# tari-project/bulletproofs-plus

Measured on AMD Instinct MI355X. Metric: 64-bit range proofs verified/sec (batch), higher is better.
Workload: dtype u32

## Files before the change

bulletproofs-plus_amd/csrc/engine.hip:

```cpp
#include <hip/hip_runtime.h>
#include <errno.h>
#include <sched.h>
#include <stdio.h>
#include <string.h>
#include <time.h>

#include <algorithm>
#include <atomic>
#include <chrono>
#include <condition_variable>
#include <deque>
#include <functional>
#include <map>
#include <set>
#include <memory>
#include <mutex>
#include <string>
#include <thread>
#include <vector>

#include "../../include/bpp.h"
#include "chain_dev.h"
#include "chain_host.h"
#include "ct.h"
// ... 323 lines not shown
    uint32_t cap = 0;
    while ((2u << cap) <= std::max<uint32_t>(max_mn, 1)) cap++;
    const uint32_t rm = std::min({rmax, (uint32_t)BPP_MAX_ROUNDS - 1, cap}), lb = lanes_lb(n_bits);
    return 1u << (rm > lb ? rm - lb : 0);
  }
  std::vector<ProofDesc> desc;
  std::vector<uint8_t> rounds_bad;
  std::vector<uint8_t> defer;
  bool any_seed = false, any_rounds_bad = false, any_defer = false, ext_challenges = false, uniform_rounds = true;
  std::vector<uint32_t> ext_status;
  DevBuf<uint32_t> d_ext_status;
  DevBuf<uint8_t> bytes, states, seeds;
  DevBuf<ProofDesc> d_desc;
  DevBuf<uint64_t> minvals;
  DevBuf<uint32_t> src_off, owner;
  DevBuf<uint32_t> idx_commit, idx_proof, status0;
  DevBuf<sc> chal, rows, scal, shr, tab;
  DevBuf<uint64_t> parts;
  bool fused_columns = false;
  uint32_t lanes_ppw = 1;
  DevBuf<int8_t> gemm_lo, gemm_hi;
  DevBuf<int32_t> gparts;
  DevBuf<sc> gemm_mult;
  bool static_gemm = false;
  uint32_t gemm_nkc = 1;
  int uniform_mn = -1;
  bool gemm_hi_ready = false;
  DevBuf<uint8_t> rng_out, weights, masks, chal_bytes;
  DevBuf<uint32_t> chain_wide;
  DevBuf<uint32_t> status, group_first, group_dlo;
  DevBuf<uint32_t> dec_spill;
  DevBuf<niels> dynpts;
  DevBuf<pniels> dyn_hi;
  MsmWork msm;
  size_t last_chunk = (size_t)-1;
  uint32_t G = 0;
  std::vector<uint32_t> h_group_first;
  PinnedBuf<uint8_t> h_rng, h_weights, h_masks;
  PinnedBuf<uint8_t> h_wide;
  PinnedBuf<uint32_t> h_status, h_ident;
  PinnedBuf<uint32_t> h_status_any;
  std::vector<uint8_t> h_status_dirty;
  const uint32_t *h_status_dirty_of = nullptr;
  bool status_settled = true;
  bool have_trace = false, phase1_done = false;
  bool status_clean = false;
  bool dev_chain_pending = false;
  bool weights_on_host = false;
  bool seeds_dirty = false, masks_dirty = false;
};

void adopt_buffers(Batch &dst, Batch &src) {
#define BPP_ADOPT(f) dst.f.swap(src.f)
  BPP_ADOPT(d_ext_status); BPP_ADOPT(bytes); BPP_ADOPT(states); BPP_ADOPT(seeds); BPP_ADOPT(d_desc); BPP_ADOPT(minvals);
  BPP_ADOPT(src_off); BPP_ADOPT(owner); BPP_ADOPT(idx_commit); BPP_ADOPT(idx_proof); BPP_ADOPT(status0); BPP_ADOPT(chal);
  BPP_ADOPT(rows); BPP_ADOPT(parts); BPP_ADOPT(gemm_lo); BPP_ADOPT(gemm_hi); BPP_ADOPT(gparts); BPP_ADOPT(gemm_mult); BPP_ADOPT(scal); BPP_ADOPT(shr); BPP_ADOPT(tab); BPP_ADOPT(rng_out); BPP_ADOPT(weights); BPP_ADOPT(chain_wide);
  BPP_ADOPT(masks); BPP_ADOPT(chal_bytes); BPP_ADOPT(status); BPP_ADOPT(group_first); BPP_ADOPT(group_dlo); BPP_ADOPT(dynpts); BPP_ADOPT(dyn_hi); BPP_ADOPT(dec_spill);
  BPP_ADOPT(msm.counts); BPP_ADOPT(msm.starts); BPP_ADOPT(msm.sorted); BPP_ADOPT(msm.order); BPP_ADOPT(msm.order_win);
  BPP_ADOPT(msm.cls_hist);
  BPP_ADOPT(msm.buckets); BPP_ADOPT(msm.Q); BPP_ADOPT(msm.W); BPP_ADOPT(msm.R); BPP_ADOPT(msm.comp32);
  BPP_ADOPT(msm.is_identity); BPP_ADOPT(msm.term_sidx); BPP_ADOPT(msm.term_pidx); BPP_ADOPT(msm.group_off);
  BPP_ADOPT(h_rng); BPP_ADOPT(h_weights); BPP_ADOPT(h_wide); BPP_ADOPT(h_status); BPP_ADOPT(h_status_any); BPP_ADOPT(h_ident); BPP_ADOPT(h_masks);
#undef BPP_ADOPT
  dst.h_status_dirty.swap(src.h_status_dirty);
  std::swap(dst.h_status_dirty_of, src.h_status_dirty_of);
  if (!src.status_settled) std::fill(dst.h_status_dirty.begin(), dst.h_status_dirty.end(), (uint8_t)1);
}

void wipe_batch_secrets(Batch &b, hipStream_t s);

}

struct PipeJob {
  uint64_t ticket = 0;
  int action = 0;
  size_t chunk = 0;
  std::shared_ptr<Params> Pp;
  uint64_t params = 0;
  UploadPlan pl;
  size_t n_items = 0;
  uint32_t t = 0;
  int rc = 0;
  std::string err;
  std::vector<uint8_t> masks, present;
  bool done = false;
};

struct PipeLane {
  bpp_ctx *child = nullptr;
  std::thread th;
  std::shared_ptr<PipeJob> job;
  bool busy = false;
};

struct Pipeline {
  std::mutex mu;
  std::condition_variable cv;
  std::mutex submit_mu;
  std::vector<std::unique_ptr<PipeLane>> lanes;
  std::map<uint64_t, std::shared_ptr<PipeJob>> tickets;
  uint64_t next_ticket = 1;
  uint32_t next_lane = 0;
  bool quit = false;
};

void pipeline_shutdown(bpp_ctx *ctx);

struct WaitHint {
  uint32_t us = 0;
  uint64_t key = 0;
};

struct bpp_ctx {
  int device = 0;
  hipStream_t stream = nullptr;
  bool own_stream = false;
  std::string err;
  std::mutex mu;
  std::multiset<uint64_t> held_params, held_precomps;
  std::map<uint64_t, std::unique_ptr<Batch>> batches;
  std::unique_ptr<Batch> spare_batch;
  PinnedBuf<uint8_t> pin_upload, pin_upload2;
  PinnedBuf<uint32_t> pin_small;
  bool profile = false;
  bool profile_light = false;
  bpp_profile prof{};
  hipEvent_t ev[16];
  bool ev_ready = false;
  hipEvent_t ev_rng;
  bool ev_rng_ready = false;
  hipEvent_t ev_wait;
  bool ev_wait_ready = false;
  WaitHint wait_hint_rng, wait_hint_end, wait_hint_prove;
  hipStream_t side_stream = nullptr;
  hipEvent_t ev_fork, ev_join;
  hipStream_t chain_stream = nullptr;
  hipEvent_t ev_chain_fork, ev_chain_done;
  DevBuf<Strobe> d_chain_t0;
  PinnedBuf<uint32_t> h_chain_zero;
  uint64_t device_chain_calls = 0, device_chain_redraws = 0, wide_chain_calls = 0;
  DevBuf<uint8_t> scratch128;
  DevBuf<uint8_t> prove_arena;
  PinnedBuf<uint8_t> prove_pin_in, prove_pin_out;
  std::vector<hipStream_t> prove_streams;
  std::vector<hipStream_t> prove_lane_streams;
  hipStream_t prove_msm_stream = nullptr;
  std::vector<hipEvent_t> prove_sync_events;
  std::vector<hipStream_t> prove_aux_streams;
  std::vector<hipEvent_t> prove_aux_events;
  std::vector<hipEvent_t> prove_events;
  bpp_prove_profile pprof{};
  struct Options {
    int transcripts_wave = -1, tables_wave = -1, side_decompress = -1, msm_c_bias = -1, msm_c_max = -1, msm_c_add = -1, msm_rc2 = -1, msm_quad = -1, msm_final_quad = -1,
        fb_threads = -1, prove_subs = -1, msm_split = -1, fused_columns = -1, prove_prio = -1, prove_fused = -1, static_gemm = -1, lazy_columns = -1, ct = -1, prove_parts = -1, prove_waves = -1, prove_fifo = -1, chain = -1, chain_test_zero = 0, wait = -1, ct_back = -1, chain_inline = -1, wide_in_lanes = -1;
  } opt;
  std::unique_ptr<Pipeline> pipe;
  std::mutex pipe_init_mu;
  uint32_t pipe_depth = 3;
};

namespace {

static uint32_t fb_threads(const bpp_ctx *ctx, uint32_t terms, const FbGeom &g) {
  if (ctx->opt.fb_threads > 0) {
    const uint32_t t = ((uint32_t)ctx->opt.fb_threads + 63u) & ~63u;
    return t > FB_THREADS ? FB_THREADS : t;
  }
  const uint32_t items = terms * g.windows;
  return items >= 4096 ? 256u : (items >= 1024 ? 128u : 64u);
}

struct OptionName {
  const char *name, *env;
  int bpp_ctx::Options::*field;
};
const OptionName kOptions[] = {
    {"transcripts_wave", "BPP_TRANSCRIPTS_WAVE", &bpp_ctx::Options::transcripts_wave},
    {"tables_wave", "BPP_TABLES_WAVE", &bpp_ctx::Options::tables_wave},
    {"side_decompress", "BPP_SIDE_DECOMPRESS", &bpp_ctx::Options::side_decompress},
    {"msm_c_bias", "BPP_MSM_C_BIAS", &bpp_ctx::Options::msm_c_bias},
    {"msm_c_max", "BPP_MSM_C_MAX", &bpp_ctx::Options::msm_c_max},
    {"msm_c_add", "BPP_MSM_C_ADD", &bpp_ctx::Options::msm_c_add},
    {"msm_rc2", "BPP_MSM_RC2", &bpp_ctx::Options::msm_rc2},
    {"msm_quad", "BPP_MSM_QUAD", &bpp_ctx::Options::msm_quad},
    {"msm_final_quad", "BPP_MSM_FINAL_QUAD", &bpp_ctx::Options::msm_final_quad},
    {"fb_threads", "BPP_FB_THREADS", &bpp_ctx::Options::fb_threads},
    {"prove_subs", "BPP_PROVE_SUBS", &bpp_ctx::Options::prove_subs},
    {"msm_split", "BPP_MSM_SPLIT", &bpp_ctx::Options::msm_split},
    {"fused_columns", "BPP_FUSED_COLUMNS", &bpp_ctx::Options::fused_columns},
    {"prove_prio", "BPP_PROVE_PRIO", &bpp_ctx::Options::prove_prio},
    {"prove_fused", "BPP_PROVE_FUSED", &bpp_ctx::Options::prove_fused},
    {"ct", "BPP_CT", &bpp_ctx::Options::ct},
    {"ct_back", "BPP_CT_BACK", &bpp_ctx::Options::ct_back},
    {"prove_parts", "BPP_PROVE_PARTS", &bpp_ctx::Options::prove_parts},
    {"prove_waves", "BPP_PROVE_WAVES", &bpp_ctx::Options::prove_waves},
    {"prove_fifo", "BPP_PROVE_FIFO", &bpp_ctx::Options::prove_fifo},
    {"static_gemm", "BPP_STATIC_GEMM", &bpp_ctx::Options::static_gemm},
    {"lazy_columns", "BPP_LAZY_COLUMNS", &bpp_ctx::Options::lazy_columns},
    {"chain", "BPP_CHAIN", &bpp_ctx::Options::chain},
    {"chain_test_zero", "BPP_CHAIN_TEST_ZERO", &bpp_ctx::Options::chain_test_zero},
    {"wait", "BPP_WAIT", &bpp_ctx::Options::wait},
    {"chain_inline", "BPP_CHAIN_INLINE", &bpp_ctx::Options::chain_inline},
    {"wide_in_lanes", "BPP_WIDE_IN_LANES", &bpp_ctx::Options::wide_in_lanes},
};
void options_from_env(bpp_ctx *c) {
  for (const OptionName &o : kOptions)
    if (const char *e = getenv(o.env)) c->opt.*(o.field) = atoi(e);
}

int fail(bpp_ctx *ctx, int code, const std::string &m, char *errbuf = nullptr, size_t len = 0) {
  if (ctx) ctx->err = m;
  set_err(errbuf, len, m);
  return code;
}

enum Mark { M_START = 0, M_TRANSCRIPTS, M_DECOMPRESS, M_SCALARS, M_WEIGHTS_IN, M_LANES, M_REDUCE, M_DIGITS, M_SORT, M_ORDER, M_ACC,
            M_BUCKET, M_FINAL, M_MASKS0, M_MASKS, M_CHAIN, M_COUNT };

struct StageTimer {
  bpp_ctx *ctx;
  bool have[16] = {false};
  explicit StageTimer(bpp_ctx *c) : ctx(c) {
    if (ctx->profile && !ctx->ev_ready) {
      for (auto &e : ctx->ev) HIP_CHECK(hipEventCreate(&e));
      ctx->ev_ready = true;
    }
  }
  void mark(int idx) {
    if (ctx->profile && idx < 16) {
      if (ctx->profile_light && idx != M_ORDER && idx != M_ACC) return;
      HIP_CHECK(hipEventRecord(ctx->ev[idx], ctx->stream));
      have[idx] = true;
    }
  }
  float between(int a, int b) {
    float ms = 0;
    if (ctx->profile && have[a] && have[b]) HIP_CHECK(hipEventElapsedTime(&ms, ctx->ev[a], ctx->ev[b]));
    return ms;
  }
};

inline uint32_t cdiv(uint32_t a, uint32_t b) { return (a + b - 1) / b; }

#define BPP_WAIT_NAP_MIN_PROOFS 4096u
inline bool wait_naps(const bpp_ctx *ctx, size_t proofs) {
  return ctx->opt.wait >= 0 ? ctx->opt.wait != 0 : proofs >= BPP_WAIT_NAP_MIN_PROOFS;
}
inline void gpu_wait_event(hipEvent_t ev, bool nap, WaitHint *wh = nullptr, uint64_t key = 0, bool tail_spin = false) {
  if (wh && wh->key != key) {
    wh->us = 0;
    wh->key = key;
  }
  uint32_t *hint = wh ? &wh->us : nullptr;
  if (!nap) {
    HIP_CHECK(hipEventSynchronize(ev));
    return;
  }
  const auto t0 = std::chrono::steady_clock::now();
  bool slept_ahead = false;
  for (;;) {
    const hipError_t e = hipEventQuery(ev);
    const long waited = (long)std::chrono::duration_cast<std::chrono::microseconds>(std::chrono::steady_clock::now() - t0).count();
    if (e == hipSuccess) {
      if (hint) *hint = *hint ? (uint32_t)((3ul * *hint + (unsigned long)waited) / 4ul) : (uint32_t)waited;
      return;
    }
    if (e != hipErrorNotReady) HIP_CHECK(e);
    if (waited < 30) continue;
    if (tail_spin && (slept_ahead || !hint || *hint <= 600)) continue;
    long nap_us;
    if (hint && !slept_ahead && *hint > 600 && waited < (long)*hint / 2) {
      nap_us = (long)*hint * (tail_spin ? 7 : 5) / 10 - waited;
      if (nap_us < 50) nap_us = 50;
      slept_ahead = true;
    } else if (slept_ahead && waited < (long)*hint * 5 / 4) {
      nap_us = 50;
    } else {
      nap_us = waited < 400 ? 50 : (waited / 8 > 400 ? 400 : waited / 8);
    }
    struct timespec ts = {0, nap_us * 1000};
    nanosleep(&ts, nullptr);
  }
}
inline void gpu_wait_stream(bpp_ctx *ctx, hipStream_t s, bool nap, WaitHint *hint = nullptr, uint64_t key = 0, bool tail_spin = false);
inline bool gpu_wait_stream_ok(bpp_ctx *ctx, hipStream_t s, bool nap) {
  try {
    gpu_wait_stream(ctx, s, nap);
    return true;
  } catch (const EngineError &) {
    (void)hipGetLastError();
    return false;
  }
}
inline void gpu_wait_stream(bpp_ctx *ctx, hipStream_t s, bool nap, WaitHint *hint, uint64_t key, bool tail_spin) {
  if (!nap) {
    HIP_CHECK(hipStreamSynchronize(s));
    return;
  }
  if (!ctx->ev_wait_ready) {
    HIP_CHECK(hipEventCreateWithFlags(&ctx->ev_wait, hipEventDisableTiming));
    ctx->ev_wait_ready = true;
  }
  HIP_CHECK(hipEventRecord(ctx->ev_wait, s));
  gpu_wait_event(ctx->ev_wait, true, hint, key, tail_spin);
}

static bool decompress_spill_enabled() {
  static const bool on = [] {
    const char *e = getenv("BPP_DECOMPRESS_SPILL");
    return e ? atoi(e) != 0 : true;
  }();
  return on;
}


#define BPP_SMALL_CALL_TERMS 20000u
uint32_t choose_window(const bpp_ctx *ctx, uint32_t group_terms, uint32_t all_terms) {
  uint32_t c = 4;
  while (c < 14 && (1u << c) * 12u <= group_terms) c++;
  const uint32_t c_max = ctx->opt.msm_c_max >= 0 ? (uint32_t)ctx->opt.msm_c_max : (group_terms < 200000u ? 11u : 14u);
  if (ctx->opt.msm_c_add > 0 && all_terms > BPP_SMALL_CALL_TERMS) c += (uint32_t)ctx->opt.msm_c_add;
  if (c > c_max && c_max >= 4) c = c_max;
  const int bias = ctx->opt.msm_c_bias >= 0 ? ctx->opt.msm_c_bias : 3;
  if (all_terms <= BPP_SMALL_CALL_TERMS) c = (uint32_t)std::max(4, std::min(11, (int)c + bias));
  return c;
}

#define BPP_SPLIT_CALL_TERMS 14000u
bool msm_wants_split(const bpp_ctx *ctx, uint32_t n_terms) {
  if (ctx->opt.msm_split >= 0) return ctx->opt.msm_split != 0 && ctx->opt.msm_quad != 0;
  return n_terms <= BPP_SPLIT_CALL_TERMS && ctx->opt.msm_quad != 0;
}
void msm_plan_alloc(bpp_ctx *ctx, MsmWork &w, const std::vector<uint32_t> &goff, bool split = false, bool copy_goff = true) {
  const uint32_t G = (uint32_t)goff.size() - 1, n = goff[G];
  uint32_t maxg = 0;
  for (uint32_t g = 0; g < G; g++) maxg = std::max(maxg, goff[g + 1] - goff[g]);
  const MsmPlan plan = msm_make_plan(choose_window(ctx, maxg, split ? n / 2 : n), G, n, split ? BPP_MSM_SPLIT_BITS : 253u);
  w.plan = plan;
  w.split = split;
  w.max_group_terms = maxg;
  const size_t nbk = (size_t)G * plan.K * plan.nb;
  w.counts.alloc(nbk);
  w.starts.alloc(nbk);
  w.sorted.alloc((size_t)n * plan.K);
  w.order.alloc(nbk);
  w.order_win.alloc(nbk);
  w.cls_hist.alloc((size_t)G * plan.K * 768);
  w.buckets.alloc(nbk);
  w.Q.alloc((size_t)G * plan.K * plan.c);
  w.W.alloc((size_t)G * plan.K);
  w.R.alloc(G);
  w.comp32.alloc((size_t)G * 32);
  w.is_identity.alloc(G);
  w.term_sidx.alloc(n);
  w.term_pidx.alloc(n);
  w.group_off.alloc(G + 1);
  HIP_CHECK(hipStreamSynchronize(ctx->stream));
  ctx->pin_small.resize(3 * (size_t)(G + 1));
  memcpy(ctx->pin_small.data(), goff.data(), (G + 1) * 4);
  if (copy_goff) HIP_CHECK(hipMemcpyAsync(w.group_off.p, ctx->pin_small.data(), (G + 1) * 4, hipMemcpyHostToDevice, ctx->stream));
}

void msm_prepare(bpp_ctx *ctx, MsmWork &w, const std::vector<uint32_t> &sidx, const std::vector<uint32_t> &pidx,
                 const std::vector<uint32_t> &goff) {
  msm_plan_alloc(ctx, w, goff);
  const uint32_t n = (uint32_t)sidx.size(), G1 = (uint32_t)goff.size();
  HIP_CHECK(hipStreamSynchronize(ctx->stream));
  ctx->pin_small.resize(3 * (size_t)G1 + 2 * (size_t)n);
  uint32_t *pin = ctx->pin_small.data() + 3 * (size_t)G1;
  memcpy(pin, sidx.data(), (size_t)n * 4);
  memcpy(pin + n, pidx.data(), (size_t)n * 4);
  HIP_CHECK(hipMemcpyAsync(w.term_sidx.p, pin, (size_t)n * 4, hipMemcpyHostToDevice, ctx->stream));
  HIP_CHECK(hipMemcpyAsync(w.term_pidx.p, pin + n, (size_t)n * 4, hipMemcpyHostToDevice, ctx->stream));
  HIP_CHECK(hipStreamSynchronize(ctx->stream));
}

void msm_run(bpp_ctx *ctx, MsmWork &w, const sc *scalars, PointTables tabs, StageTimer *tm) {
  const MsmPlan plan = w.plan;
  hipStream_t s = ctx->stream;
  const uint32_t per_group = plan.K * plan.nb;
  const bool small = w.split || (ctx->opt.msm_quad >= 0 ? ctx->opt.msm_quad != 0 : (size_t)plan.G * per_group <= 100000);
  const bool narrow = !small && w.max_group_terms <= BPP_SORT_SMALL_GROUP_TERMS;
  if (narrow) {
    const uint32_t dig_cap = msm_prelude_dig_cap(plan, w.max_group_terms, BPP_SORT_THREADS_SMALL);
    hipLaunchKernelGGL(k_msm_prelude<BPP_SORT_THREADS_SMALL>, dim3(8 * cdiv(plan.G, 8) * plan.K), dim3(BPP_SORT_THREADS_SMALL), msm_prelude_lds(plan, dig_cap), s,
                       scalars, w.term_sidx.p, w.term_pidx.p, w.group_off.p, plan, dig_cap, w.counts.p, w.starts.p, w.sorted.p, w.order_win.p, w.cls_hist.p);
    hipLaunchKernelGGL(k_msm_order<BPP_SORT_THREADS_SMALL>, dim3(plan.G), dim3(BPP_SORT_THREADS_SMALL), 0, s, w.counts.p, w.order_win.p, w.cls_hist.p, plan,
                       w.order.p);
  } else {
    const uint32_t dig_cap = msm_prelude_dig_cap(plan, w.max_group_terms);
    hipLaunchKernelGGL(k_msm_prelude<BPP_SORT_THREADS>, dim3(8 * cdiv(plan.G, 8) * plan.K), dim3(BPP_SORT_THREADS), msm_prelude_lds(plan, dig_cap), s, scalars,
                       w.term_sidx.p, w.term_pidx.p, w.group_off.p, plan, dig_cap, w.counts.p, w.starts.p, w.sorted.p, w.order_win.p, w.cls_hist.p);
    hipLaunchKernelGGL(k_msm_order<BPP_SORT_THREADS>, dim3(plan.G), dim3(BPP_SORT_THREADS), 0, s, w.counts.p, w.order_win.p, w.cls_hist.p, plan, w.order.p);
  }
  if (tm) tm->mark(M_ORDER);
  if (small)
    hipLaunchKernelGGL(k_msm_accumulate_quad, dim3(cdiv(plan.G * per_group, 16)), dim3(64), 0, s, w.sorted.p, w.starts.p,
                       w.counts.p, w.order.p, tabs, plan.G * per_group, w.buckets.p);
  else
    hipLaunchKernelGGL(k_msm_accumulate, dim3(8 * cdiv(plan.G, 8) * cdiv(per_group, 64)), dim3(64), 0, s, w.sorted.p, w.starts.p,
                       w.counts.p, w.order.p, tabs, per_group, plan.G, w.buckets.p);
  if (tm) tm->mark(M_ACC);
  if (plan.c <= 11 && small) {
    hipLaunchKernelGGL(k_msm_window_rc_quad, dim3(plan.G * plan.K), dim3(1024), 0, s, w.buckets.p, w.counts.p, plan, w.W.p);
  } else if (plan.nb <= 256 && ctx->opt.msm_rc2 != 0) {
    hipLaunchKernelGGL(k_msm_window_rc2, dim3(cdiv(plan.G * plan.K, 2)), dim3(64), 0, s, w.buckets.p, w.counts.p, plan, plan.G * plan.K, w.W.p);
  } else if (plan.c <= 11) {
    hipLaunchKernelGGL(k_msm_window_rc, dim3(plan.G * plan.K), dim3(64), 0, s, w.buckets.p, w.counts.p, plan, w.W.p);
  } else {
    hipLaunchKernelGGL(k_msm_bitsum, dim3(plan.c, plan.K, plan.G), dim3(64), 0, s, w.buckets.p, w.counts.p, plan, w.Q.p);
    hipLaunchKernelGGL(k_msm_window, dim3(cdiv(plan.G * plan.K, 64)), dim3(64), 0, s, w.Q.p, plan, w.W.p);
  }
  if (tm) tm->mark(M_BUCKET);
  {
    if (ctx->opt.msm_final_quad != 0)
      hipLaunchKernelGGL(k_msm_final_quad, dim3(cdiv(plan.G, 16)), dim3(64), 0, s, w.W.p, plan, w.R.p, w.is_identity.p);
    else
      hipLaunchKernelGGL(k_msm_final, dim3(cdiv(plan.G, 64)), dim3(64), 0, s, w.W.p, plan, w.R.p, w.is_identity.p);
  }
  if (tm) tm->mark(M_FINAL);
  HIP_CHECK(hipGetLastError());
}

uint32_t decompress_to_device(bpp_ctx *ctx, const uint8_t *pts32, size_t n, niels *out) {
  DevBuf<uint8_t> d_in;
  DevBuf<uint32_t> d_bad;
  d_in.alloc(n * 32);
  d_bad.alloc(1);
  HIP_CHECK(hipMemcpyAsync(d_in.p, pts32, n * 32, hipMemcpyHostToDevice, ctx->stream));
  HIP_CHECK(hipMemsetAsync(d_bad.p, 0, 4, ctx->stream));
  hipLaunchKernelGGL(k_decompress_plain, dim3(cdiv((uint32_t)n, 64)), dim3(64), 0, ctx->stream, d_in.p, (uint32_t)n, out,
                     d_bad.p);
  uint32_t bad = 0;
  HIP_CHECK(hipMemcpyAsync(&bad, d_bad.p, 4, hipMemcpyDeviceToHost, ctx->stream));
  HIP_CHECK(hipStreamSynchronize(ctx->stream));
  return bad;
}

int msm_host_entry(bpp_ctx *ctx, const niels *tab_a, uint32_t n_a, const uint8_t *static_scalars32, size_t n_static,
                   const uint8_t *dyn_scalars32, const uint8_t *dyn_points32, size_t n_dyn,
                   const uint32_t *group_off_in, size_t n_groups, uint8_t *out32) {
  const size_t n = n_static + n_dyn;
  std::vector<uint8_t> sb(n * 32 + 32);
  if (n_static) memcpy(sb.data(), static_scalars32, n_static * 32);
  if (n_dyn) memcpy(sb.data() + n_static * 32, dyn_scalars32, n_dyn * 32);
  for (size_t i = 0; i < n; i++)
    if (!sc_is_canonical(sb.data() + 32 * i)) return fail(ctx, BPP_ERR_INVALID_ARGUMENT, "scalar is not canonical");
  if (n == 0 || n_groups == 0) {
    for (size_t g = 0; g < (n_groups ? n_groups : 1); g++) memset(out32 + 32 * g, 0, 32);
    return BPP_OK;
  }
  DevBuf<sc> d_sc;
  DevBuf<niels> d_dyn;
  d_sc.alloc(n);
  d_dyn.alloc(n_dyn);
  HIP_CHECK(hipMemcpyAsync(d_sc.p, sb.data(), n * 32, hipMemcpyHostToDevice, ctx->stream));
  if (n_dyn) {
    uint32_t bad = decompress_to_device(ctx, dyn_points32, n_dyn, d_dyn.p);
    if (bad) return fail(ctx, BPP_ERR_INVALID_ARGUMENT, "point is not a canonical ristretto255 encoding");
  }
  std::vector<uint32_t> sidx(n), pidx(n), goff;
  for (size_t i = 0; i < n; i++) {
    sidx[i] = (uint32_t)i;
    pidx[i] = (i < n_static) ? (uint32_t)i : (uint32_t)(n_a + (i - n_static));
  }
  if (group_off_in) {
    goff.assign(group_off_in, group_off_in + n_groups + 1);
  } else {
    goff = {0u, (uint32_t)n};
  }
  MsmWork w;
  msm_prepare(ctx, w, sidx, pidx, goff);
  PointTables tabs{tab_a, d_dyn.p, n_a, nullptr, nullptr};
  msm_run(ctx, w, d_sc.p, tabs, nullptr);
  hipLaunchKernelGGL(k_compress_ge, dim3(cdiv(w.plan.G, 64)), dim3(64), 0, ctx->stream, w.R.p, w.plan.G, w.comp32.p);
  HIP_CHECK(hipMemcpyAsync(out32, w.comp32.p, 32 * (goff.size() - 1), hipMemcpyDeviceToHost, ctx->stream));
  HIP_CHECK(hipStreamSynchronize(ctx->stream));
  return BPP_OK;
}

}

extern "C" {

int bpp_ctx_create_on_stream(bpp_ctx **out, int device_id, void *hip_stream) {
  if (!out) return BPP_ERR_BAD_HANDLE;
  *out = nullptr;
  int count = 0;
  if (hipGetDeviceCount(&count) != hipSuccess || count <= 0 || device_id < 0 || device_id >= count) return BPP_ERR_NO_DEVICE;
  hipDeviceProp_t prop;
  if (hipGetDeviceProperties(&prop, device_id) != hipSuccess) return BPP_ERR_NO_DEVICE;
  if (strncmp(prop.gcnArchName, "gfx950", 6) != 0) return BPP_ERR_NO_DEVICE;
  if (hipSetDevice(device_id) != hipSuccess) return BPP_ERR_NO_DEVICE;
  bpp_ctx *c = new bpp_ctx();
  c->device = device_id;
  options_from_env(c);
  if (hip_stream) {
    c->stream = (hipStream_t)hip_stream;
  } else {
    if (hipStreamCreateWithFlags(&c->stream, hipStreamNonBlocking) != hipSuccess) {
      delete c;
      return BPP_ERR_ENGINE;
    }
    c->own_stream = true;
  }
  {
    DeviceState &D = device_state(device_id);
    std::lock_guard<std::mutex> lk(D.mu);
    D.contexts++;
    D.contexts_peak = std::max(D.contexts_peak, D.contexts);
    const uint32_t q = runtime_hw_queues();
    if (D.contexts > q) {
      char note[256];
      snprintf(note, sizeof(note), "note: %u contexts on %u hardware queues (GPU_MAX_HW_QUEUES=%u, read by the HIP runtime at start-up): "
               "streams beyond that share queues and their kernels serialise; see INTEGRATION.md, runtime preconditions", D.contexts, q, q);
      c->err = note;
      D.warned = true;
    }
    if (!D.env_note.empty()) c->err = D.env_note;
  }
  *out = c;
  return BPP_OK;
}

int bpp_ctx_create(bpp_ctx **out, int device_id) { return bpp_ctx_create_on_stream(out, device_id, nullptr); }

void bpp_ctx_destroy(bpp_ctx *ctx) {
  if (!ctx) return;
  (void)hipSetDevice(ctx->device);
  pipeline_shutdown(ctx);
  { std::lock_guard<std::mutex> lk(ctx->mu); }
  (void)hipStreamSynchronize(ctx->stream);
  for (auto &kv : ctx->batches) wipe_batch_secrets(*kv.second, ctx->stream);
  (void)hipStreamSynchronize(ctx->stream);
  ctx->batches.clear();
  ctx->spare_batch.reset();
  for (uint64_t h : ctx->held_precomps) (void)precomp_registry().release(h);
  for (uint64_t h : ctx->held_params) (void)params_registry().release(h);
  if (ctx->ev_ready)
    for (auto &e : ctx->ev) (void)hipEventDestroy(e);
  if (ctx->ev_rng_ready) (void)hipEventDestroy(ctx->ev_rng);
  if (ctx->ev_wait_ready) (void)hipEventDestroy(ctx->ev_wait);
  if (ctx->side_stream) {
    (void)hipStreamSynchronize(ctx->side_stream);
    (void)hipStreamDestroy(ctx->side_stream);
    (void)hipEventDestroy(ctx->ev_fork);
    (void)hipEventDestroy(ctx->ev_join);
  }
  if (ctx->chain_stream) {
    (void)hipStreamSynchronize(ctx->chain_stream);
    (void)hipStreamDestroy(ctx->chain_stream);
// ... 1881 lines not shown
```

bulletproofs-plus_amd/csrc/msm.h:

```cpp
#pragma once
#include "point.h"
#include "recode.h"
#include "scalar.h"

namespace bpp {

struct PointTables {
  const niels *tab_a;
  const niels *tab_b;
  uint32_t n_a;
  const niels *tab_a_hi;
  const struct pniels *tab_b_hi;
};
struct pniels {
  fe yplusx, yminusx, xy2d, z2;
};
__device__ const uint32_t BPP_FE_TWO[10] = {2, 0, 0, 0, 0, 0, 0, 0, 0, 0};
__device__ __forceinline__ const niels *point_ptr(const PointTables &t, uint32_t idx) {
  return idx < t.n_a ? (t.tab_a + idx) : (t.tab_b + (idx - t.n_a));
}


#ifndef BPP_SORT_THREADS
#define BPP_SORT_THREADS 1024
// ... 8 lines not shown
  return msm_digit_at(h, plan, k);
}
template <uint32_t T>
__global__ void __launch_bounds__(T) k_msm_prelude(const sc *__restrict__ scalars, const uint32_t *__restrict__ term_sidx,
                                                   const uint32_t *__restrict__ term_pidx, const uint32_t *__restrict__ group_off,
                                                   MsmPlan plan, uint32_t dig_cap, uint32_t *__restrict__ counts,
                                                   uint32_t *__restrict__ starts, uint32_t *__restrict__ sorted,
                                                   uint32_t *__restrict__ order_win, uint32_t *__restrict__ cls_hist) {
  extern __shared__ uint32_t lds[];
  const uint32_t tid = threadIdx.x, nb = plan.nb, K = plan.K;
  const uint32_t xcd = blockIdx.x & 7u, j = blockIdx.x >> 3;
  const uint32_t g = xcd + 8u * (j / K), k = j % K;
  if (g >= plan.G) return;
  uint32_t *hist = lds, *cur = lds + nb;
  int16_t *dcache = (int16_t *)(lds + 2 * nb);
  __shared__ uint32_t part[T];
  __shared__ uint32_t cls_n[256], cls_start[256], cls_cur[256];
  const uint32_t t0 = group_off[g], ng = group_off[g + 1] - t0;
  const uint32_t region = t0 * K + k * ng;
  for (uint32_t q = tid; q < nb; q += T) hist[q] = 0;
  if (tid < 256) cls_n[tid] = cls_cur[tid] = 0;
  __syncthreads();
  for (uint32_t i0 = tid; i0 < ng; i0 += 8 * T) {
    uint32_t si[8];
    int32_t d[8];
#pragma unroll
    for (int u = 0; u < 8; u++) si[u] = (i0 + u * T < ng) ? term_sidx[t0 + i0 + u * T] : 0xffffffffu;
#pragma unroll
    for (int u = 0; u < 8; u++) d[u] = si[u] != 0xffffffffu ? msm_term_digit(scalars, si[u], plan, k) : 0;
#pragma unroll
    for (int u = 0; u < 8; u++) {
      const uint32_t i = i0 + u * T;
      if (i < ng) {
        if (i < dig_cap) dcache[i] = (int16_t)d[u];
        if (d[u]) atomicAdd(&hist[(uint32_t)(d[u] < 0 ? -d[u] : d[u]) - 1], 1u);
      }
    }
  }
  __syncthreads();
  const uint32_t per = (nb + T - 1u) / T;
  const uint32_t a = tid * per < nb ? tid * per : nb, b = (a + per < nb) ? a + per : nb;
  uint32_t sum = 0;
  for (uint32_t q = a; q < b; q++) sum += hist[q];
  part[tid] = sum;
  __syncthreads();
  for (uint32_t off = 1; off < T; off <<= 1) {
    uint32_t v = (tid >= off) ? part[tid - off] : 0;
    __syncthreads();
    part[tid] += v;
    __syncthreads();
  }
  uint32_t run = (tid == 0) ? 0 : part[tid - 1];
  const size_t bbase = ((size_t)g * K + k) * nb;
  for (uint32_t q = a; q < b; q++) {
    const uint32_t cnt = hist[q];
    counts[bbase + q] = cnt;
    starts[bbase + q] = region + run;
    cur[q] = run;
    run += cnt;
    atomicAdd(&cls_n[cnt < 255u ? cnt : 255u], 1u);
  }
  __syncthreads();
  for (uint32_t i0 = tid; i0 < ng; i0 += 8 * T) {
    int32_t d[8];
    uint32_t pi[8];
#pragma unroll
    for (int u = 0; u < 8; u++) {
      const uint32_t i = i0 + u * T;
      const bool in = i < ng;
      pi[u] = in ? term_pidx[t0 + i] : 0u;
      d[u] = !in ? 0 : (i < dig_cap ? (int32_t)dcache[i] : msm_term_digit(scalars, term_sidx[t0 + i], plan, k));
    }
#pragma unroll
    for (int u = 0; u < 8; u++)
      if (d[u]) {
        const uint32_t pos = atomicAdd(&cur[(uint32_t)(d[u] < 0 ? -d[u] : d[u]) - 1], 1u);
        sorted[region + pos] = pi[u] | (d[u] < 0 ? 0x80000000u : 0u);
      }
  }
  uint32_t *gh = cls_hist + (size_t)g * K * 768;
  if (tid < 256) part[tid] = cls_n[tid];
  __syncthreads();
  for (uint32_t off = 1; off < 256; off <<= 1) {
    uint32_t v = (tid < 256 && tid + off < 256) ? part[tid + off] : 0;
    __syncthreads();
    if (tid < 256) part[tid] += v;
    __syncthreads();
  }
  if (tid < 256) {
    cls_start[tid] = part[tid] - cls_n[tid];
    gh[k * 768 + tid] = cls_n[tid];
    gh[k * 768 + 256 + tid] = cls_start[tid];
  }
  __syncthreads();
  for (uint32_t q = a; q < b; q++) {
    const uint32_t cnt = hist[q], cls = cnt < 255u ? cnt : 255u;
    const uint32_t pos = cls_start[cls] + atomicAdd(&cls_cur[cls], 1u);
    order_win[bbase + pos] = (uint32_t)(bbase + q);
  }
}

template <uint32_t T>
__global__ void __launch_bounds__(T) k_msm_order(const uint32_t *__restrict__ counts, const uint32_t *__restrict__ order_win,
                                                 uint32_t *cls_hist, MsmPlan plan, uint32_t *__restrict__ order) {
  const uint32_t tid = threadIdx.x, g = blockIdx.x, nb = plan.nb, K = plan.K;
  __shared__ uint32_t part[256];
  uint32_t *gh = cls_hist + (size_t)g * K * 768;
  const size_t gbase = (size_t)g * K * nb;
  uint32_t tot = 0;
  if (tid < 256) {
    for (uint32_t kk = 0; kk < K; kk++) tot += gh[kk * 768 + tid];
    part[tid] = tot;
  }
  __syncthreads();
  for (uint32_t off = 1; off < 256; off <<= 1) {
    uint32_t v = (tid < 256 && tid + off < 256) ? part[tid + off] : 0;
    __syncthreads();
    if (tid < 256) part[tid] += v;
    __syncthreads();
  }
  if (tid < 256) {
    uint32_t running = part[tid] - tot;
    for (uint32_t kk = 0; kk < K; kk++) {
      gh[kk * 768 + 512 + tid] = running - gh[kk * 768 + 256 + tid];
      running += gh[kk * 768 + tid];
    }
  }
  __syncthreads();
  const uint32_t n_all = K * nb;
  for (uint32_t i0 = tid; i0 < n_all; i0 += 4 * T) {
    uint32_t bk[4], cn[4];
#pragma unroll
    for (int u = 0; u < 4; u++) bk[u] = i0 + u * T < n_all ? order_win[gbase + i0 + u * T] : 0xffffffffu;
#pragma unroll
    for (int u = 0; u < 4; u++) cn[u] = bk[u] != 0xffffffffu ? counts[bk[u]] : 0u;
#pragma unroll
    for (int u = 0; u < 4; u++)
      if (bk[u] != 0xffffffffu) {
        const uint32_t i = i0 + u * T, kk = i >> (plan.c - 1u), q = i & (nb - 1u);
        order[gbase + (uint32_t)(q + gh[kk * 768 + 512 + (cn[u] < 255u ? cn[u] : 255u)])] = bk[u];
      }
  }
}
inline uint32_t msm_prelude_dig_cap(const MsmPlan &plan, uint32_t max_group_terms, uint32_t threads = BPP_SORT_THREADS) {
  const uint32_t fixed = 2u * plan.nb * 4u + (threads + 3u * 256u) * 4u;
  const uint32_t room = fixed + 1024u < 65536u ? (65536u - 1024u - fixed) / 2u : 0u;
  return max_group_terms < room ? max_group_terms : room;
}
inline size_t msm_prelude_lds(const MsmPlan &plan, uint32_t dig_cap) { return (size_t)2 * plan.nb * 4 + (size_t)((dig_cap + 1u) & ~1u) * 2; }

#ifndef BPP_ACC_WAVES
#define BPP_ACC_WAVES 3
#endif
__global__ void __launch_bounds__(64, BPP_ACC_WAVES) k_msm_accumulate(const uint32_t *__restrict__ sorted,
                                                       const uint32_t *__restrict__ starts,
                                                       const uint32_t *__restrict__ counts,
                                                       const uint32_t *__restrict__ order, PointTables tabs,
                                                       uint32_t per_group, uint32_t G, ge *__restrict__ buckets) {
  const uint32_t xcd = blockIdx.x & 7u, j = blockIdx.x >> 3;
  const uint32_t bpg = (per_group + 63u) / 64u;
  const uint32_t g = xcd + 8u * (j / bpg);
  const uint32_t slot = (j % bpg) * 64u + threadIdx.x;
  if (g >= G || slot >= per_group) return;
  const uint32_t bkt = order[(size_t)g * per_group + slot];
  const uint32_t a = starts[bkt], n = counts[bkt];
  if (n == 0) return;
  uint32_t e = sorted[a];
  niels q;
  niels_load_swapped(q, point_ptr(tabs, e & 0x7fffffffu), (e >> 31) != 0);
  ge acc;
  ge_from_niels_first(acc, q);
  fe_fence(acc.X);
  fe_fence(acc.Y);
  fe_fence(acc.T);
  if (n > 1) {
    e = sorted[a + 1];
    niels_load_swapped(q, point_ptr(tabs, e & 0x7fffffffu), (e >> 31) != 0);
  }
  uint32_t i = 1;
  while (i < n) {
    uint32_t e2 = e;
    niels q2;
    if (i + 1 < n) {
      e2 = sorted[a + i + 1];
      niels_load_swapped(q2, point_ptr(tabs, e2 & 0x7fffffffu), (e2 >> 31) != 0);
    }
    ge_madd_swapped(acc, acc, q, (e >> 31) != 0);
    if (++i >= n) break;
    if (i + 1 < n) {
      e = sorted[a + i + 1];
      niels_load_swapped(q, point_ptr(tabs, e & 0x7fffffffu), (e >> 31) != 0);
    }
    ge_madd_swapped(acc, acc, q2, (e2 >> 31) != 0);
    ++i;
  }
  buckets[bkt] = acc;
}

__global__ void __launch_bounds__(64) k_msm_window_rc(const ge *__restrict__ buckets, const uint32_t *__restrict__ counts,
                                                      MsmPlan plan, ge *__restrict__ W) {
  const uint32_t gk = blockIdx.x, lane = threadIdx.x;
  const uint32_t nb = plan.nb, lb = plan.c - 1;
  const uint32_t lBc = lb / 2, Bc = 1u << lBc, A = nb >> lBc;
  const size_t base = (size_t)gk * nb;
  __shared__ ge red[64];
  ge acc;
  ge_identity(acc);
  const bool is_row = lane < 32;
  const uint32_t idx = is_row ? lane : lane - 32;
  if (is_row ? (idx < A) : (idx < Bc)) {
    const uint32_t cnt = is_row ? Bc : A;
    for (uint32_t q = 0; q < cnt; q++) {
      const uint32_t j0 = is_row ? (Bc * idx + q) : (Bc * q + idx);
      if (counts[base + j0]) {
        const ge x = buckets[base + j0];
        ge_add(acc, acc, x);
      }
    }
  }
  red[lane] = acc;
  __syncthreads();
  const uint32_t half_n = is_row ? A : Bc;
  for (uint32_t off = 1; off < 32; off <<= 1) {
    ge y2;
    const bool act = idx + off < half_n;
    if (act) y2 = red[lane + off];
    __syncthreads();
    if (act) {
      ge_add(acc, acc, y2);
      red[lane] = acc;
    }
    __syncthreads();
  }
  if (is_row ? (idx == 0 || idx >= A) : (idx >= Bc)) ge_identity(acc);
  red[lane] = acc;
  __syncthreads();
  for (uint32_t off = 16; off >= 1; off >>= 1) {
    if (idx < off) {
      ge x = red[lane], y2 = red[lane + off];
      ge_add(x, x, y2);
      red[lane] = x;
    }
    __syncthreads();
  }
  if (lane == 0) {
    ge rows = red[0];
    const ge cols = red[32];
    if (lBc) ge_dbl_n(rows, rows, (int)lBc);
    ge_add(rows, rows, cols);
    W[gk] = rows;
  }
}

__global__ void __launch_bounds__(64) k_msm_window_rc2(const ge *__restrict__ buckets, const uint32_t *__restrict__ counts, MsmPlan plan,
                                                       uint32_t n_windows, ge *__restrict__ W) {
  const uint32_t lane = threadIdx.x;
  const uint32_t nb = plan.nb, lb = plan.c - 1;
  const uint32_t lBc = lb / 2, Bc = 1u << lBc, A = nb >> lBc;
  const bool is_row = lane < 32;
  const uint32_t sub = (lane >> 4) & 1u, idx = lane & 15u;
  const uint32_t gk = blockIdx.x * 2u + sub;
  const bool live = gk < n_windows;
  const size_t base = (size_t)gk * nb;
  __shared__ ge red[64];
  ge acc;
  ge_identity(acc);
  if (live && (is_row ? (idx < A) : (idx < Bc))) {
    const uint32_t cnt = is_row ? Bc : A;
    for (uint32_t q = 0; q < cnt; q++) {
      const uint32_t j0 = is_row ? (Bc * idx + q) : (Bc * q + idx);
      if (counts[base + j0]) {
        const ge x = buckets[base + j0];
        ge_add(acc, acc, x);
      }
    }
  }
  red[lane] = acc;
  __syncthreads();
  const uint32_t half_n = is_row ? A : Bc;
  for (uint32_t off = 1; off < 16; off <<= 1) {
    ge y2;
    const bool act = idx + off < half_n;
    if (act) y2 = red[lane + off];
    __syncthreads();
    if (act) {
      ge_add(acc, acc, y2);
      red[lane] = acc;
    }
    __syncthreads();
  }
  if (is_row ? (idx == 0 || idx >= A) : (idx >= Bc)) ge_identity(acc);
  red[lane] = acc;
  __syncthreads();
  for (uint32_t off = 8; off >= 1; off >>= 1) {
    if (idx < off) {
      ge x = red[lane], y2 = red[lane + off];
      ge_add(x, x, y2);
      red[lane] = x;
    }
    __syncthreads();
  }
  if (is_row && idx == 0 && live) {
    ge rows = red[lane];
    const ge cols = red[lane + 32];
    if (lBc) ge_dbl_n(rows, rows, (int)lBc);
    ge_add(rows, rows, cols);
    W[gk] = rows;
  }
}

__global__ void __launch_bounds__(64) k_msm_bitsum(const ge *__restrict__ buckets, const uint32_t *__restrict__ counts,
                                                   MsmPlan plan, ge *__restrict__ Q ) {
  const uint32_t b = blockIdx.x, k = blockIdx.y, g = blockIdx.z, lane = threadIdx.x;
  const uint32_t nb = plan.nb;
  const size_t base = ((size_t)g * plan.K + k) * nb;
  __shared__ ge red[64];
  ge acc;
  ge_identity(acc);
  for (uint32_t j = lane; j < nb; j += 64) {
    if ((((j + 1) >> b) & 1u) && counts[base + j] != 0) {
      const ge q = buckets[base + j];
      ge_add(acc, acc, q);
    }
  }
  red[lane] = acc;
  __syncthreads();
  for (uint32_t off = 32; off >= 1; off >>= 1) {
    if (lane < off) {
      ge x = red[lane], y2 = red[lane + off];
      ge_add(x, x, y2);
      red[lane] = x;
    }
    __syncthreads();
  }
  if (lane == 0) Q[((size_t)g * plan.K + k) * plan.c + b] = red[0];
}

__global__ void __launch_bounds__(64) k_msm_window(const ge *__restrict__ Q, MsmPlan plan, ge *__restrict__ W) {
  const uint32_t i = blockIdx.x * blockDim.x + threadIdx.x;
  if (i >= plan.G * plan.K) return;
  const ge *q = Q + (size_t)i * plan.c;
  ge acc = q[plan.c - 1];
  for (int b = (int)plan.c - 2; b >= 0; b--) {
    ge_dbl(acc, acc);
    const ge x = q[b];
    ge_add(acc, acc, x);
  }
  W[i] = acc;
}
// ... 420 lines not shown
```

Before: 27.74 million.

## Fuse MSM bucket ordering into the accumulate kernel for large MSMs

For the non-small MSM path, the separate k_msm_order kernel is skipped. A new k_msm_accumulate_ordered kernel computes each slot's bucket directly from the per-window class histograms. It builds a suffix sum over count classes in LDS, binary-searches the slot's class, then walks the windows to find the position in order_win. This removes one kernel launch and the global write and read of the order array, but every accumulate block redoes the histogram reduction and extra gathers. The path is on by default (fuse=-1) and can be turned off with BPP_FUSE=0.

```diff
diff --git a/bulletproofs-plus_amd/csrc/engine.hip b/bulletproofs-plus_amd/csrc/engine.hip
--- a/bulletproofs-plus_amd/csrc/engine.hip
+++ b/bulletproofs-plus_amd/csrc/engine.hip
@@ -499,7 +499,7 @@
   bpp_prove_profile pprof{};
   struct Options {
     int transcripts_wave = -1, tables_wave = -1, side_decompress = -1, msm_c_bias = -1, msm_c_max = -1, msm_c_add = -1, msm_rc2 = -1, msm_quad = -1, msm_final_quad = -1,
-        fb_threads = -1, prove_subs = -1, msm_split = -1, fused_columns = -1, prove_prio = -1, prove_fused = -1, static_gemm = -1, lazy_columns = -1, ct = -1, prove_parts = -1, prove_waves = -1, prove_fifo = -1, chain = -1, chain_test_zero = 0, wait = -1, ct_back = -1, chain_inline = -1, wide_in_lanes = -1;
+        fb_threads = -1, prove_subs = -1, msm_split = -1, fused_columns = -1, prove_prio = -1, prove_fused = -1, static_gemm = -1, lazy_columns = -1, ct = -1, prove_parts = -1, prove_waves = -1, prove_fifo = -1, chain = -1, chain_test_zero = 0, wait = -1, ct_back = -1, chain_inline = -1, wide_in_lanes = -1, fuse = -1;
   } opt;
   std::unique_ptr<Pipeline> pipe;
   std::mutex pipe_init_mu;
@@ -549,6 +549,7 @@
     {"wait", "BPP_WAIT", &bpp_ctx::Options::wait},
     {"chain_inline", "BPP_CHAIN_INLINE", &bpp_ctx::Options::chain_inline},
     {"wide_in_lanes", "BPP_WIDE_IN_LANES", &bpp_ctx::Options::wide_in_lanes},
+    {"fuse", "BPP_FUSE", &bpp_ctx::Options::fuse},
 };
 void options_from_env(bpp_ctx *c) {
   for (const OptionName &o : kOptions)
@@ -728,22 +729,28 @@
   const uint32_t per_group = plan.K * plan.nb;
   const bool small = w.split || (ctx->opt.msm_quad >= 0 ? ctx->opt.msm_quad != 0 : (size_t)plan.G * per_group <= 100000);
   const bool narrow = !small && w.max_group_terms <= BPP_SORT_SMALL_GROUP_TERMS;
+  const bool order_in_acc = !small && ctx->opt.fuse != 0;
   if (narrow) {
     const uint32_t dig_cap = msm_prelude_dig_cap(plan, w.max_group_terms, BPP_SORT_THREADS_SMALL);
     hipLaunchKernelGGL(k_msm_prelude<BPP_SORT_THREADS_SMALL>, dim3(8 * cdiv(plan.G, 8) * plan.K), dim3(BPP_SORT_THREADS_SMALL), msm_prelude_lds(plan, dig_cap), s,
                        scalars, w.term_sidx.p, w.term_pidx.p, w.group_off.p, plan, dig_cap, w.counts.p, w.starts.p, w.sorted.p, w.order_win.p, w.cls_hist.p);
-    hipLaunchKernelGGL(k_msm_order<BPP_SORT_THREADS_SMALL>, dim3(plan.G), dim3(BPP_SORT_THREADS_SMALL), 0, s, w.counts.p, w.order_win.p, w.cls_hist.p, plan,
-                       w.order.p);
+    if (!order_in_acc)
+      hipLaunchKernelGGL(k_msm_order<BPP_SORT_THREADS_SMALL>, dim3(plan.G), dim3(BPP_SORT_THREADS_SMALL), 0, s, w.counts.p, w.order_win.p, w.cls_hist.p,
+                         plan, w.order.p);
   } else {
     const uint32_t dig_cap = msm_prelude_dig_cap(plan, w.max_group_terms);
     hipLaunchKernelGGL(k_msm_prelude<BPP_SORT_THREADS>, dim3(8 * cdiv(plan.G, 8) * plan.K), dim3(BPP_SORT_THREADS), msm_prelude_lds(plan, dig_cap), s, scalars,
                        w.term_sidx.p, w.term_pidx.p, w.group_off.p, plan, dig_cap, w.counts.p, w.starts.p, w.sorted.p, w.order_win.p, w.cls_hist.p);
-    hipLaunchKernelGGL(k_msm_order<BPP_SORT_THREADS>, dim3(plan.G), dim3(BPP_SORT_THREADS), 0, s, w.counts.p, w.order_win.p, w.cls_hist.p, plan, w.order.p);
+    if (!order_in_acc)
+      hipLaunchKernelGGL(k_msm_order<BPP_SORT_THREADS>, dim3(plan.G), dim3(BPP_SORT_THREADS), 0, s, w.counts.p, w.order_win.p, w.cls_hist.p, plan, w.order.p);
   }
   if (tm) tm->mark(M_ORDER);
   if (small)
     hipLaunchKernelGGL(k_msm_accumulate_quad, dim3(cdiv(plan.G * per_group, 16)), dim3(64), 0, s, w.sorted.p, w.starts.p,
                        w.counts.p, w.order.p, tabs, plan.G * per_group, w.buckets.p);
+  else if (order_in_acc)
+    hipLaunchKernelGGL(k_msm_accumulate_ordered, dim3(8 * cdiv(plan.G, 8) * cdiv(per_group, 64)), dim3(64), 0, s, w.sorted.p, w.starts.p,
+                       w.counts.p, w.order_win.p, w.cls_hist.p, plan, tabs, w.buckets.p);
   else
     hipLaunchKernelGGL(k_msm_accumulate, dim3(8 * cdiv(plan.G, 8) * cdiv(per_group, 64)), dim3(64), 0, s, w.sorted.p, w.starts.p,
                        w.counts.p, w.order.p, tabs, per_group, plan.G, w.buckets.p);
diff --git a/bulletproofs-plus_amd/csrc/msm.h b/bulletproofs-plus_amd/csrc/msm.h
--- a/bulletproofs-plus_amd/csrc/msm.h
+++ b/bulletproofs-plus_amd/csrc/msm.h
@@ -184,17 +184,9 @@
 #ifndef BPP_ACC_WAVES
 #define BPP_ACC_WAVES 3
 #endif
-__global__ void __launch_bounds__(64, BPP_ACC_WAVES) k_msm_accumulate(const uint32_t *__restrict__ sorted,
-                                                       const uint32_t *__restrict__ starts,
-                                                       const uint32_t *__restrict__ counts,
-                                                       const uint32_t *__restrict__ order, PointTables tabs,
-                                                       uint32_t per_group, uint32_t G, ge *__restrict__ buckets) {
-  const uint32_t xcd = blockIdx.x & 7u, j = blockIdx.x >> 3;
-  const uint32_t bpg = (per_group + 63u) / 64u;
-  const uint32_t g = xcd + 8u * (j / bpg);
-  const uint32_t slot = (j % bpg) * 64u + threadIdx.x;
-  if (g >= G || slot >= per_group) return;
-  const uint32_t bkt = order[(size_t)g * per_group + slot];
+__device__ __forceinline__ void msm_bucket_sum(const uint32_t *__restrict__ sorted, const uint32_t *__restrict__ starts,
+                                               const uint32_t *__restrict__ counts, const PointTables &tabs, uint32_t bkt,
+                                               ge *__restrict__ buckets) {
   const uint32_t a = starts[bkt], n = counts[bkt];
   if (n == 0) return;
   uint32_t e = sorted[a];
@@ -227,6 +219,77 @@
     ++i;
   }
   buckets[bkt] = acc;
+}
+__global__ void __launch_bounds__(64, BPP_ACC_WAVES) k_msm_accumulate(const uint32_t *__restrict__ sorted,
+                                                       const uint32_t *__restrict__ starts,
+                                                       const uint32_t *__restrict__ counts,
+                                                       const uint32_t *__restrict__ order, PointTables tabs,
+                                                       uint32_t per_group, uint32_t G, ge *__restrict__ buckets) {
+  const uint32_t xcd = blockIdx.x & 7u, j = blockIdx.x >> 3;
+  const uint32_t bpg = (per_group + 63u) / 64u;
+  const uint32_t g = xcd + 8u * (j / bpg);
+  const uint32_t slot = (j % bpg) * 64u + threadIdx.x;
+  if (g >= G || slot >= per_group) return;
+  msm_bucket_sum(sorted, starts, counts, tabs, order[(size_t)g * per_group + slot], buckets);
+}
+
+__global__ void __launch_bounds__(64, BPP_ACC_WAVES) k_msm_accumulate_ordered(const uint32_t *__restrict__ sorted,
+                                                               const uint32_t *__restrict__ starts,
+                                                               const uint32_t *__restrict__ counts,
+                                                               const uint32_t *__restrict__ order_win,
+                                                               const uint32_t *__restrict__ cls_hist, MsmPlan plan,
+                                                               PointTables tabs, ge *__restrict__ buckets) {
+  const uint32_t K = plan.K, per_group = K * plan.nb, lane = threadIdx.x;
+  const uint32_t xcd = blockIdx.x & 7u, j = blockIdx.x >> 3;
+  const uint32_t bpg = (per_group + 63u) / 64u;
+  const uint32_t g = xcd + 8u * (j / bpg);
+  const uint32_t slot = (j % bpg) * 64u + lane;
+  if (g >= plan.G) return;
+  __shared__ uint32_t suf[257];
+  const uint32_t *gh = cls_hist + (size_t)g * K * 768;
+  uint4 t = make_uint4(0u, 0u, 0u, 0u);
+#pragma unroll 8
+  for (uint32_t kk = 0; kk < K; kk++) {
+    const uint4 v = *(const uint4 *)(gh + kk * 768u + 4u * lane);
+    t.x += v.x;
+    t.y += v.y;
+    t.z += v.z;
+    t.w += v.w;
+  }
+  const uint32_t own = t.x + t.y + t.z + t.w;
+  uint32_t hi = own;
+#pragma unroll
+  for (uint32_t off = 1; off < 64; off <<= 1) {
+    const uint32_t v = __shfl_down(hi, off, 64);
+    if (lane + off < 64u) hi += v;
+  }
+  const uint32_t above = hi - own;
+  suf[4u * lane + 3u] = above + t.w;
+  suf[4u * lane + 2u] = above + t.w + t.z;
+  suf[4u * lane + 1u] = above + t.w + t.z + t.y;
+  suf[4u * lane] = hi;
+  if (lane == 0) suf[256] = 0;
+  __syncthreads();
+  if (slot >= per_group) return;
+  uint32_t c = 0;
+#pragma unroll
+  for (uint32_t step = 128; step; step >>= 1)
+    if (suf[c + step] > slot) c += step;
+  uint32_t r = slot - suf[c + 1], kk = K;
+  for (uint32_t k0 = 0; k0 < K && kk == K; k0 += 8) {
+    uint32_t n[8];
+#pragma unroll
+    for (uint32_t u = 0; u < 8; u++) n[u] = k0 + u < K ? gh[(k0 + u) * 768u + c] : 0xffffffffu;
+#pragma unroll
+    for (uint32_t u = 0; u < 8; u++)
+      if (kk == K) {
+        if (r < n[u]) kk = k0 + u;
+        else r -= n[u];
+      }
+  }
+  if (kk == K) return;
+  const uint32_t pos = gh[kk * 768u + 256u + c] + r;
+  msm_bucket_sum(sorted, starts, counts, tabs, order_win[(size_t)g * per_group + kk * plan.nb + pos], buckets);
 }
 
 __global__ void __launch_bounds__(64) k_msm_window_rc(const ge *__restrict__ buckets, const uint32_t *__restrict__ counts,
```

After: 27.71 million, median of 6. About the same (-0.1%).
